# GaloisInc/pure-zlib

Hardware: AMD Instinct MI355X
Metric: decompressed GiB/s (whole node) on 64K level-6 zlib blobs; bit-exact vs ref (higher is better)
Workload: dtype u8

## Files before the change

pure_zlib_amd/csrc/inflate_core.h:

```cpp
#pragma once
#include <stddef.h>
#include <stdint.h>

#include "wave.h"

#if defined(PZG_PROFILE) && PZG_DEVICE_PASS && defined(PZG_PROFILE_HDR)
#define PZG_T0(var) const uint64_t var = __builtin_amdgcn_s_memtime()
#define PZG_ACC(slot, var) ((slot) >= 8 && (slot) <= 11 ? (void)var : (void)(prof[slot] += __builtin_amdgcn_s_memtime() - var))
#define PZG_ACCW(slot, var) ((void)var)
#define PZG_HACC(slot, var) prof[slot] += __builtin_amdgcn_s_memtime() - var
#elif defined(PZG_PROFILE) && PZG_DEVICE_PASS && defined(PZG_PROFILE_HOT)
#define PZG_T0(var) const uint64_t var = __builtin_amdgcn_s_memtime()
#define PZG_ACC(slot, var) ((slot) >= 8 && (slot) <= 11 ? (void)var : (void)(prof[slot] += __builtin_amdgcn_s_memtime() - var))
#define PZG_ACCW(slot, var) ((void)var)
#define PZG_HACC(slot, var)
#define PZG_HOT_ACC(slot, var) prof[slot] += __builtin_amdgcn_s_memtime() - var
#elif defined(PZG_PROFILE) && PZG_DEVICE_PASS
#define PZG_T0(var) const uint64_t var = __builtin_amdgcn_s_memtime()
#define PZG_ACC(slot, var) prof[slot] += __builtin_amdgcn_s_memtime() - var
#define PZG_ACCW(slot, var) (__builtin_amdgcn_s_waitcnt(0xc07f), prof[slot] += __builtin_amdgcn_s_memtime() - var)
#define PZG_HACC(slot, var)
#else
#define PZG_HACC(slot, var)
#define PZG_T0(var)
#define PZG_ACC(slot, var)
#define PZG_ACCW(slot, var)
#endif
#if defined(PZG_MARKS) && PZG_DEVICE_PASS
#define PZG_MARK(name) asm volatile("; ##MARK " name)
#else
#define PZG_MARK(name)
#endif
#ifndef PZG_HOT_ACC
#define PZG_HOT_ACC(slot, var)
#endif
#if defined(PZG_PROFILE) && PZG_DEVICE_PASS && defined(PZG_PROFILE_HOT)
#define PZG_SEQ_T0(var) uint64_t var = __builtin_amdgcn_s_memtime()
#define PZG_SEQ_ACC(slot, var) (__builtin_amdgcn_s_waitcnt(0x0070), prof[slot] += __builtin_amdgcn_s_memtime() - var, var = __builtin_amdgcn_s_memtime())
#else
#define PZG_SEQ_T0(var)
#define PZG_SEQ_ACC(slot, var)
#endif

#if defined(PZG_STATS) && !PZG_DEVICE_PASS
struct PzgStats { unsigned long long v[32]; };
extern PzgStats pzg_stats;
#define PZG_STAT(i, n) (pzg_stats.v[i] += (unsigned long long)(n))
#else
#define PZG_STAT(i, n) ((void)0)
#endif
#ifndef PZG_RES_HOT_LOOP
#define PZG_RES_HOT_LOOP 1
#endif
#ifndef PZG_WALK_UNROLL
#define PZG_WALK_UNROLL 8
#endif
#ifndef PZG_HOT_ALIGN
#define PZG_HOT_ALIGN 6
#endif
#ifndef PZG_WALK_EXIT_ALIGN
#define PZG_WALK_EXIT_ALIGN 2
#endif
#define PZG_STR2(x) #x
#define PZG_STR(x) PZG_STR2(x)

namespace pzg {

enum : int32_t {
    ST_OK = 0,
    ST_TRUNCATED = 1,
    ST_HDR_FCHECK = 2,
    ST_HDR_METHOD = 3,
    ST_HDR_WINDOW = 4,
    ST_FMT_LEN_NLEN = 5,
    ST_FMT_BTYPE = 6,
    ST_HUFF_BUILD = 7,
    ST_HUFF_EMPTY_TREE = 8,
    ST_HUFF_EMPTY_BRANCH = 9,
    ST_CHECKSUM = 10,
    ST_BAD_DISTANCE = 11,
    ST_BAD_LITLEN_SYMBOL = 12,
    ST_BAD_DIST_SYMBOL = 13,
    ST_OUT_TOO_SMALL = 14,
    ST_GZIP_HEADER = 18,
    ST_GZIP_ISIZE = 19,
    ST_DICT = 20,
    ST_SEGMENT = 21,
    ST_NEED_INPUT = 101,
    ST_OUT_FULL = 102,
    ST_RETRY_FULL_RING = 100,
    ST_BUNDLE_TODO = 103
};

enum { TREE_CODELEN = 0, TREE_LITLEN = 1, TREE_DIST = 2 };

#ifndef PZG_LIT_BITS
#define PZG_LIT_BITS 8
#endif
constexpr int LIT_BITS = PZG_LIT_BITS;
#ifndef PZG_SUB_ENTRIES
#define PZG_SUB_ENTRIES 252
#endif
constexpr uint32_t SUB_ENTRIES = PZG_SUB_ENTRIES;
static_assert(SUB_ENTRIES <= 256u, "K_SUB entries hold an 8-bit pool index");
#ifndef PZG_SUB_BITS_MAX
#define PZG_SUB_BITS_MAX 5
#endif
constexpr uint32_t SUB_BITS_MAX = PZG_SUB_BITS_MAX;
#ifndef PZG_SUB_MIN
#define PZG_SUB_MIN 3
#endif
constexpr uint32_t SUB_MIN_PREFIXES = PZG_SUB_MIN;
constexpr int DIST_BITS = 8;
constexpr int CL_BITS = 7;
constexpr uint32_t ADLER_MOD = 65521u;

constexpr int MAX_LIT_SYMS = 288;
constexpr int MAX_DIST_SYMS = 32 + 138;
constexpr int MAX_LENS = 288 + 32 + 138;

enum : uint32_t {
    K_LIT = 0,
    K_BASE = 1,
    K_EOB = 2,
    K_LONG = 3,
    K_EMPTY_BRANCH = 4,
    K_EMPTY_TREE = 5,
    K_BADSYM = 6,
// ... 1537 lines not shown
    template <bool FX>
    PZG_FN bool fill_queue()
    {
        while (__builtin_expect(br.window2_ok(), 1)) {
            if (__builtin_expect(window_append2<FX>(), 0)) return true;
            if (qn >= QHIGH) return false;
        }
        if (RES) {
            do {
                if (!br.window_ok() || window_append<FX>()) return true;
            } while (qn < QHIGH);
            return false;
        }
        do {
            if (window_append2<FX, true>()) return true;
        } while (qn < QHIGH);
        return false;
    }

    enum : uint32_t { HL_GENERAL = 1, HL_WINDOW = 2 };
    template <bool FX, int SUB>
    PZG_FN uint32_t hot_loop(LaneVec<uint32_t> &TK0, LaneVec<uint32_t> &TK1, uint64_t &S0, uint64_t &S1, uint32_t &k0, uint32_t &k1)
    {
        uint32_t why;
#if PZG_DEVICE_PASS && PZG_HOT_ALIGN
        asm volatile(".p2align " PZG_STR(PZG_HOT_ALIGN));
#endif
        for (;;) {
            if (qn < QHIGH) {
                if (__builtin_expect(!br.window2_ok(), 0)) {
                    why = HL_GENERAL;
                    break;
                }
                PZG_T0(thw);
                LaneVec<uint32_t> TB0, TB1;
                window2_decode<FX, false, SUB>(TB0, TK0, TB1, TK1);
                S0 = 0;
                S1 = 0;
                k1 = 0;
                PZG_STAT(0, 1);
                k0 = walk_half(TB0, 0u, S0);
                why = HL_WINDOW;
                if (__builtin_expect(k0 >= 64u, 0)) break;
                k1 = walk_half(TB1, k0, S1);
                if (__builtin_expect(k1 >= 64u, 0)) break;
                const uint32_t nt0 = popc64(S0), nt1 = popc64(S1);
                if (__builtin_expect((qn + nt0) + nt1 > QCAP, 0)) break;
                PZG_STAT(1, nt0 + nt1);
                queue_append(TK0, S0, nt0, TK1, S1, nt1);
                br.drop_short(k1 + 128u);
                PZG_HOT_ACC(8, thw);
                continue;
            }
            PZG_T0(the);
            if (emit_body<true>() != ST_OK) {
                why = HL_GENERAL;
                break;
            }
            PZG_HOT_ACC(9, the);
        }
#if PZG_DEVICE_PASS
        asm volatile("" : "+s"(why));
#endif
        return why;
    }


    static constexpr bool STRIPS = true;
#ifndef PZG_STRIP_TMAX
#define PZG_STRIP_TMAX 192
#endif
#ifndef PZG_STRIP_BACK
#define PZG_STRIP_BACK 1024
#endif
    static constexpr uint32_t STRIP_TMAX = PZG_STRIP_TMAX;
    static_assert(STRIP_TMAX % 16u == 0u && STRIP_TMAX <= 1008u, "region geometry");
    static constexpr bool SEQ_LROVF = STRIP_TMAX > 240u;
#ifndef PZG_SEQ_GROUP
#define PZG_SEQ_GROUP 8
#endif
#ifndef PZG_TOP_MOVES
#define PZG_TOP_MOVES 1
#endif
    static constexpr uint32_t SEQ_G = PZG_SEQ_GROUP;
    static constexpr uint32_t REG_LITA = 32u;
    static constexpr uint32_t REG_RECA = (REG_LITA + STRIP_TMAX + 4u * SEQ_G + 31u) & ~31u;
#ifndef PZG_REG_PAD
#define PZG_REG_PAD 0
#endif
    static constexpr uint32_t REG_BYTES = ((REG_RECA + 4u * STRIP_TMAX + 63u) & ~63u) + PZG_REG_PAD;
    static constexpr uint32_t PROF_OFF = 64u * (REG_BYTES / 4u) + 128u;
    static constexpr uint32_t STRIP_WORDS = PROF_OFF + 80u;
    static constexpr uint32_t PROF_MAGIC = 0x51DF0A7Eu;
#ifndef PZG_STRIP_PROFILE
#define PZG_STRIP_PROFILE 1
#endif
    static constexpr bool STRIP_PROFILE = PZG_STRIP_PROFILE != 0 && !RES;
#ifndef PZG_PROF_LIKELY
#define PZG_PROF_LIKELY(x) __builtin_expect(!!(x), 0)
#endif
    static constexpr uint32_t PROF_TGT = STRIP_TMAX * 3u / 4u;
#ifndef PZG_PROF_CMIN
#define PZG_PROF_CMIN 512
#endif
    static constexpr uint32_t PROF_CMIN = PZG_PROF_CMIN;
    static constexpr uint32_t PROF_HEAD = 2048u;
    static constexpr uint32_t STRIP_BACK = PZG_STRIP_BACK;
#ifndef PZG_STRIP_BACK_MIN
#define PZG_STRIP_BACK_MIN 256
#endif
    static constexpr uint32_t STRIP_BACK_MIN = PZG_STRIP_BACK_MIN < PZG_STRIP_BACK ? PZG_STRIP_BACK_MIN : PZG_STRIP_BACK;
    static constexpr uint32_t STRIP_BACK_DOWN = 32u, STRIP_BACK_UP = 256u;
#ifndef PZG_STRIP_CMIN
#define PZG_STRIP_CMIN 64
#endif
    static constexpr uint32_t STRIP_CMIN = PZG_STRIP_CMIN;
#ifndef PZG_STRIP_BACK_PER_C
#define PZG_STRIP_BACK_PER_C 2
#endif
    static constexpr uint32_t STRIP_BACK_PER_C = PZG_STRIP_BACK_PER_C;
#ifndef PZG_STRIP_ROUNDS
#define PZG_STRIP_ROUNDS 6
#endif
    static constexpr uint32_t STRIP_ROUNDS = PZG_STRIP_ROUNDS;
    static constexpr int STRIP_NA = -2;
    PZG_FN static constexpr uint32_t reg_rec(uint32_t k) { return k * (REG_BYTES / 4u) + REG_RECA / 4u; }
    PZG_FN static constexpr uint32_t reg_lit(uint32_t k) { return k * REG_BYTES + REG_LITA; }

    static constexpr uint32_t SEQ_NOMATCH = 0x80000000u;
    PZG_FN static uint32_t seq_nl(uint32_t rec) { return (rec >> 23) & 255u; }
    PZG_FN static uint32_t seq_len(uint32_t rec) { return (int32_t)rec < 0 ? 0u : ((rec >> 15) & 255u) + 3u; }
    PZG_FN static uint32_t seq_dist(uint32_t rec) { return (rec & 0x7fffu) + 1u; }

    PZG_FN uint32_t strip_load(uint32_t i) const
    {
#if PZG_DEVICE_PASS
        return __hip_atomic_load(strip + i, __ATOMIC_RELAXED, __HIP_MEMORY_SCOPE_AGENT);
#else
        return strip[i];
#endif
    }
    PZG_FN uint32_t lit_load32(uint32_t off) const
    {
        const uint8_t *p = reinterpret_cast<const uint8_t *>(strip) + off;
#if PZG_DEVICE_PASS
        return __hip_atomic_load(reinterpret_cast<const uint32_t *>(p), __ATOMIC_RELAXED, __HIP_MEMORY_SCOPE_AGENT);
#else
        uint32_t v;
        __builtin_memcpy(&v, p, 4);
        return v;
#endif
    }
    PZG_FN uint8_t lit_load8(uint32_t off) const
    {
        const uint8_t *p = reinterpret_cast<const uint8_t *>(strip) + off;
#if PZG_DEVICE_PASS
        return __hip_atomic_load(p, __ATOMIC_RELAXED, __HIP_MEMORY_SCOPE_AGENT);
#else
        return *p;
#endif
    }
    PZG_FN void strip_fence() const
    {
#if PZG_DEVICE_PASS
        asm volatile("s_waitcnt vmcnt(0)" ::: "memory");
#endif
// ... 756 lines not shown
        PZG_HOT_ACC(10, tsc);
        PZG_T0(tse);
        for (;;) {
            const uint32_t why = seq_hot();
            if (why == SQ_DONE) break;
            if (why == SQ_FLUSH) {
                flush_to(op & ~(uint64_t)15u);
                continue;
            }
            const int se = seq_solo();
            if (se) return se;
        }
        PZG_HOT_ACC(11, tse);
        strip_kill_window_state();
        return ST_OK;
    }
    PZG_FN void strip_kill_window_state()
    {
        PZG_LANES_BEGIN(j)
            PZG_LV(QT, j) = 0u;
            PZG_LV(pendF0, j) = 0;
            PZG_LV(pendF1, j) = 0;
        PZG_LANES_END
    }
#undef PZG_SR

#ifndef PZG_SEQ_GLIM
#define PZG_SEQ_GLIM 768
#endif
#ifndef PZG_SEQ_CAP
#define PZG_SEQ_CAP 32
#endif
    static constexpr uint32_t SEQ_GLIM = PZG_SEQ_GLIM;
    static constexpr uint32_t SEQ_CAP = PZG_SEQ_CAP;
    static_assert(SEQ_GLIM + SEQ_CAP + 3u + 128u <= 1024u && SEQ_GLIM >= 255u + SEQ_CAP, "far sources end a cache line or more below `flushed`; one sequence always fits");
    enum : uint32_t { SQ_OK = 0, SQ_DONE = 1, SQ_SOLO = 2, SQ_FLUSH = 3 };

    static constexpr uint32_t RING_OFF = (uint32_t)offsetof(WaveLds<RING_BITS>, ring);
    static constexpr uint32_t DUMP_REL = (uint32_t)(offsetof(WaveLds<RING_BITS>, dump) - offsetof(WaveLds<RING_BITS>, ring));
    struct Quad {
        uint8_t b[4];
    };
    template <uint32_t OFF>
    PZG_FN void lds_copy4x2(const LaneVec<uint32_t> &SM, const LaneVec<uint32_t> &DM, uint64_t m0, uint64_t m1)
    {
#if PZG_DEVICE_PASS
        static_assert(RING_OFF % 4u == 0u && OFF % 8u == 0u, "aligned dwords");
        uint32_t a, sh, d0, d1, d2, q0, q1, y0, y1;
        uint64_t sv;
        asm volatile("s_mov_b64 %9, exec\n\t"
                     "s_mov_b64 exec, %12\n\t"
                     "v_and_b32 %0, -4, %10\n\t"
                     "v_lshlrev_b32 %1, 3, %10\n\t"
                     "ds_read_b32 %2, %0 offset:%c14\n\tds_read_b32 %3, %0 offset:%c15\n\tds_read_b32 %4, %0 offset:%c16\n\t"
                     "s_waitcnt lgkmcnt(0)\n\t"
                     "v_alignbit_b32 %5, %3, %2, %1\n\t"
                     "v_alignbit_b32 %6, %4, %3, %1\n\t"
                     "v_lshrrev_b32 %7, 8, %5\n\t"
                     "v_lshrrev_b32 %8, 8, %6\n\t"
                     "s_mov_b64 exec, %13\n\t"
                     "ds_write_b8_d16_hi %11, %8 offset:%c24\n\tds_write_b8_d16_hi %11, %6 offset:%c23\n\tds_write_b8 %11, %8 offset:%c22\n\tds_write_b8 %11, %6 offset:%c21\n\t"
                     "s_mov_b64 exec, %12\n\t"
                     "ds_write_b8_d16_hi %11, %7 offset:%c20\n\tds_write_b8_d16_hi %11, %5 offset:%c19\n\tds_write_b8 %11, %7 offset:%c18\n\tds_write_b8 %11, %5 offset:%c17\n\t"
                     "s_mov_b64 exec, %9"
                     : "=&v"(a), "=&v"(sh), "=&v"(d0), "=&v"(d1), "=&v"(d2), "=&v"(q0), "=&v"(q1), "=&v"(y0), "=&v"(y1), "=&s"(sv)
                     : "v"(SM.v), "v"(DM.v), "s"(m0), "s"(m1), "n"(RING_OFF + OFF), "n"(RING_OFF + OFF + 4u), "n"(RING_OFF + OFF + 8u),
                       "n"(RING_OFF + OFF), "n"(RING_OFF + OFF + 1u), "n"(RING_OFF + OFF + 2u), "n"(RING_OFF + OFF + 3u), "n"(RING_OFF + OFF + 4u),
                       "n"(RING_OFF + OFF + 5u), "n"(RING_OFF + OFF + 6u), "n"(RING_OFF + OFF + 7u)
                     : "memory");
#else
        LaneVec<Quad> A, B;
        for (uint32_t j = 0; j < 64u; ++j)
            for (uint32_t t = 0; t < 4u; ++t) {
                if ((m0 >> j) & 1u) A.v[j].b[t] = L.ring[SM.v[j] + OFF + t];
                if ((m1 >> j) & 1u) B.v[j].b[t] = L.ring[SM.v[j] + OFF + 4u + t];
            }
        for (uint32_t j = 0; j < 64u; ++j)
            for (uint32_t t = 4u; t-- > 0u;) {
                if ((m1 >> j) & 1u) L.ring[DM.v[j] + OFF + 4u + t] = B.v[j].b[t];
                if ((m0 >> j) & 1u) L.ring[DM.v[j] + OFF + t] = A.v[j].b[t];
            }
#endif
    }
    PZG_FN void lds_copy_tail(const LaneVec<uint32_t> &ST, const LaneVec<uint32_t> &DT, uint64_t m4, const LaneVec<uint32_t> &S3,
                              const LaneVec<uint32_t> &D3, uint64_t m3)
    {
#if PZG_DEVICE_PASS
        uint32_t sa, da, a, sh, d0, d1, q, y;
        uint64_t sv;
        asm volatile("s_mov_b64 %8, exec\n\t"
                     "s_or_b64 exec, %13, %14\n\t"
                     "v_cndmask_b32_e64 %0, %11, %9, %13\n\t"
                     "v_cndmask_b32_e64 %1, %12, %10, %13\n\t"
                     "v_and_b32 %2, -4, %0\n\t"
                     "v_lshlrev_b32 %3, 3, %0\n\t"
                     "ds_read_b32 %4, %2 offset:%c15\n\tds_read_b32 %5, %2 offset:%c19\n\t"
                     "s_waitcnt lgkmcnt(0)\n\t"
                     "v_alignbit_b32 %6, %5, %4, %3\n\t"
                     "v_lshrrev_b32 %7, 8, %6\n\t"
                     "s_mov_b64 exec, %13\n\t"
                     "ds_write_b8_d16_hi %1, %7 offset:%c18\n\t"
                     "s_or_b64 exec, %13, %14\n\t"
                     "ds_write_b8_d16_hi %1, %6 offset:%c17\n\tds_write_b8 %1, %7 offset:%c16\n\tds_write_b8 %1, %6 offset:%c15\n\t"
                     "s_mov_b64 exec, %8"
                     : "=&v"(sa), "=&v"(da), "=&v"(a), "=&v"(sh), "=&v"(d0), "=&v"(d1), "=&v"(q), "=&v"(y), "=&s"(sv)
                     : "v"(ST.v), "v"(DT.v), "v"(S3.v), "v"(D3.v), "s"(m4), "s"(m3), "n"(RING_OFF), "n"(RING_OFF + 1u), "n"(RING_OFF + 2u), "n"(RING_OFF + 3u),
                       "n"(RING_OFF + 4u)
                     : "memory", "scc");
#else
        LaneVec<Quad> A, B;
        for (uint32_t j = 0; j < 64u; ++j)
            for (uint32_t t = 0; t < 4u; ++t) {
                if ((m4 >> j) & 1u) A.v[j].b[t] = L.ring[ST.v[j] + t];
                if (((m3 >> j) & 1u) && t < 3u) B.v[j].b[t] = L.ring[S3.v[j] + t];
            }
        for (uint32_t j = 0; j < 64u; ++j)
            for (uint32_t t = 4u; t-- > 0u;) {
                if (((m3 >> j) & 1u) && t < 3u) L.ring[D3.v[j] + t] = B.v[j].b[t];
                if ((m4 >> j) & 1u) L.ring[DT.v[j] + t] = A.v[j].b[t];
            }
#endif
    }
    PZG_FN void lds_put_bytes(const LaneVec<uint32_t> &A, const LaneVec<uint32_t> &X, uint64_t m0, uint64_t m1, uint64_t m2, uint64_t m3)
    {
#if PZG_DEVICE_PASS
        uint32_t y;
        uint64_t sv;
        asm volatile("s_mov_b64 %1, exec\n\t"
                     "s_mov_b64 exec, %7\n\t"
                     "v_lshrrev_b32 %0, 8, %3\n\t"
                     "ds_write_b8_d16_hi %2, %0 offset:%c11\n\t"
                     "s_mov_b64 exec, %6\n\t"
                     "ds_write_b8_d16_hi %2, %3 offset:%c10\n\t"
                     "s_mov_b64 exec, %5\n\t"
                     "v_lshrrev_b32 %0, 8, %3\n\t"
                     "ds_write_b8 %2, %0 offset:%c9\n\t"
                     "s_mov_b64 exec, %4\n\t"
                     "ds_write_b8 %2, %3 offset:%c8\n\t"
                     "s_mov_b64 exec, %1"
                     : "=&v"(y), "=&s"(sv)
                     : "v"(A.v), "v"(X.v), "s"(m0), "s"(m1), "s"(m2), "s"(m3), "n"(RING_OFF), "n"(RING_OFF + 1u), "n"(RING_OFF + 2u), "n"(RING_OFF + 3u)
                     : "memory");
#else
        for (uint32_t j = 0; j < 64u; ++j) {
            if ((m3 >> j) & 1u) L.ring[A.v[j] + 3u] = (uint8_t)(X.v[j] >> 24);
            if ((m2 >> j) & 1u) L.ring[A.v[j] + 2u] = (uint8_t)(X.v[j] >> 16);
            if ((m1 >> j) & 1u) L.ring[A.v[j] + 1u] = (uint8_t)(X.v[j] >> 8);
            if ((m0 >> j) & 1u) L.ring[A.v[j]] = (uint8_t)X.v[j];
        }
#endif
    }
    PZG_FN void lds_put_dword(const LaneVec<uint32_t> &A, const LaneVec<uint32_t> &X, uint64_t m)
    {
#if PZG_DEVICE_PASS
        uint32_t y;
        uint64_t sv;
        asm volatile("s_mov_b64 %1, exec\n\t"
                     "s_mov_b64 exec, %4\n\t"
                     "v_lshrrev_b32 %0, 8, %3\n\t"
                     "ds_write_b8_d16_hi %2, %0 offset:%c8\n\tds_write_b8_d16_hi %2, %3 offset:%c7\n\tds_write_b8 %2, %0 offset:%c6\n\tds_write_b8 %2, %3 offset:%c5\n\t"
                     "s_mov_b64 exec, %1"
                     : "=&v"(y), "=&s"(sv)
                     : "v"(A.v), "v"(X.v), "s"(m), "n"(RING_OFF), "n"(RING_OFF + 1u), "n"(RING_OFF + 2u), "n"(RING_OFF + 3u)
                     : "memory");
#else
        lds_put_bytes(A, X, m, m, m, m);
#endif
    }
    PZG_FN uint32_t far_off(uint32_t op32, uint32_t fdelta, uint32_t rel) const
    {
        return RES_HIST ? (op32 + rel) & HIST_MASK : 32768u + fdelta + rel;
    }
    PZG_FN uint32_t far_load32(uint32_t off) const
    {
#if PZG_DEVICE_PASS
        if (RES_HIST)
            return __hip_atomic_load(reinterpret_cast<const uint32_t *>(far_base + off), __ATOMIC_RELAXED, __HIP_MEMORY_SCOPE_AGENT);
#endif
        uint32_t v;
        __builtin_memcpy(&v, far_base + off, 4);
        return v;
    }
    PZG_FN uint8_t far_load8(uint32_t off) const
    {
#if PZG_DEVICE_PASS
        if (RES_HIST) return __hip_atomic_load(far_base + off, __ATOMIC_RELAXED, __HIP_MEMORY_SCOPE_AGENT);
#endif
        return far_base[off];
    }
    static constexpr uint32_t FAR_DUMMY = RES_HIST ? 0u : FAR_IDLE;
    struct SeqCopy {
        LaneVec<uint32_t> SM, DM, LEN, NB, ST, DT;
        uint64_t norm4, norm3, slow;
    };
    template <uint32_t T>
    PZG_FN void seq_copy_trips(const SeqCopy &c, uint64_t m4)
    {
        if constexpr (T < SEQ_CAP / 8u) {
            LaneVec<bool> A0, A1;
            PZG_LANES_BEGIN(j)
                PZG_LV(A0, j) = 2u * T < PZG_LV(c.NB, j);
                PZG_LV(A1, j) = 2u * T + 1u < PZG_LV(c.NB, j);
            PZG_LANES_END
            const uint64_t m0 = m4 & lanes_ballot(A0), m1 = m4 & lanes_ballot(A1);
            if (m0 == 0ull) return;
            lds_copy4x2<8u * T>(c.SM, c.DM, m0, m1);
            PZG_STAT(26, 1);
            seq_copy_trips<T + 1u>(c, m4);
        }
    }
    PZG_FN void seq_copy(const SeqCopy &c, uint64_t rdy)
    {
        const uint64_t m4 = rdy & c.norm4, m3 = rdy & c.norm3, sl = rdy & c.slow;
        if (m4 != 0ull) seq_copy_trips<0u>(c, m4);
        lds_copy_tail(c.ST, c.DT, m4, c.SM, c.DM, m3);
        if (__builtin_expect(sl != 0ull, 0)) {
            LaneVec<bool> ACT;
            LaneVec<uint32_t> X;
            for (uint32_t i = 0;; ++i) {
                PZG_LANES_BEGIN(j)
                    PZG_LV(ACT, j) = lane_bit(sl, j) & (i < PZG_LV(c.LEN, j));
                PZG_LANES_END
                if (lanes_ballot(ACT) == 0ull) break;
                PZG_LANES_BEGIN(j)
                    PZG_LV(X, j) = L.ring[(PZG_LV(c.SM, j) + i) & RMASK];
                PZG_LANES_END
                PZG_LANES_BEGIN(j)
                    ring_store(PZG_LV(ACT, j), (PZG_LV(c.DM, j) + i) & RMASK, (uint8_t)PZG_LV(X, j), j);
                PZG_LANES_END
                PZG_STAT(27, 1);
            }
        }
    }

    PZG_FN uint32_t seq_group()
    {
        const uint32_t n = s_qn;
        if (n == 0u) return SQ_DONE;
        if (__builtin_expect((uint32_t)(op - flushed) >= FLUSH_AT, 0)) {
            const uint64_t to = flushed + ((uint32_t)(op - flushed) & ~1023u);
            if (!out_aligned() || to > cap) return SQ_FLUSH;
            flush_span<true>(to);
        }
        PZG_SEQ_T0(tq);
        PZG_MARK("g.begin");
        const uint32_t op32 = (uint32_t)op;
        uint32_t op_hi = (uint32_t)(op >> 32);
#if PZG_DEVICE_PASS
        asm("" : "+s"(op_hi));
#endif
        const uint32_t hist = (op_hi | (op32 >> 20)) ? 0x100000u : op32 + (RING_BITS == 15 ? hist_extra : 0u);
        LaneVec<uint32_t> NL, LEN, DIST, ENDX, MO;
        PZG_LANES_BEGIN(j)
            const uint32_t rec = PZG_LV(QTN, j);
            const bool valid = j < n;
            const uint32_t nl = valid ? seq_nl(rec) : 0u, len = valid ? seq_len(rec) : 0u;
            PZG_LV(NL, j) = nl;
            PZG_LV(LEN, j) = len;
            PZG_LV(DIST, j) = seq_dist(rec);
            PZG_LV(ENDX, j) = (nl + len) | (nl << 16);
        PZG_LANES_END
        lanes_iscan_add(ENDX);
        LaneVec<bool> OVER, BAD, MIX, HASM;
        PZG_LANES_BEGIN(j)
            const uint32_t end = PZG_LV(ENDX, j) & 0xffffu, len = PZG_LV(LEN, j), m = end - len;
            PZG_LV(MO, j) = m;
            PZG_LV(OVER, j) = end > SEQ_GLIM;
            PZG_LV(HASM, j) = len != 0u;
            PZG_LV(BAD, j) = PZG_LV(DIST, j) > hist + m;
            PZG_LV(MIX, j) = (int32_t)(m - PZG_LV(DIST, j)) < (int32_t)(SEQ_GLIM - RING);
        PZG_LANES_END
        const uint64_t stopm = lanes_ballot(OVER) | (lanes_ballot(HASM) & (lanes_ballot(BAD) | (RING_BITS == 15 ? lanes_ballot(MIX) : 0ull)));
        const uint32_t v0 = stopm ? ctz64(stopm) : n;
        const uint32_t v = v0 < n ? v0 : n;
        if (__builtin_expect(v == 0u, 0)) return SQ_SOLO;
        const uint32_t endv = lane_get(ENDX, v - 1u), run = endv & 0xffffu, lend_v = endv >> 16;
        const uint64_t taken = v >= 64u ? ~0ull : bit_field_mask(v, 0u);
        PZG_STAT(20, 1);
        PZG_STAT(21, v);
        PZG_STAT(22, run);
        SeqCopy c;
        LaneVec<uint32_t> SEND;
        LaneVec<bool> B_LEN, B_NEAR, B_WD, B_WS, B_D16, B_OV, B_D4, B_BIG, B_L4, B_L3;
        PZG_LANES_BEGIN(j)
            const uint32_t len = PZG_LV(LEN, j), dist = PZG_LV(DIST, j), m = PZG_LV(MO, j);
            const int32_t srcr = (int32_t)(m - dist);
            const uint32_t dm = (op32 + m) & RMASK, sm = (dm - dist) & RMASK;
            PZG_LV(c.LEN, j) = len;
            PZG_LV(c.DM, j) = dm;
            PZG_LV(c.SM, j) = sm;
            PZG_LV(c.NB, j) = (len - 1u) >> 2;
            PZG_LV(c.ST, j) = sm + len - 4u;
            PZG_LV(c.DT, j) = dm + len - 4u;
            PZG_LV(B_LEN, j) = len != 0u;
            PZG_LV(B_NEAR, j) = srcr >= (int32_t)(run - RING);
            PZG_LV(B_WD, j) = dm + len > RING;
            PZG_LV(B_WS, j) = sm + len > RING;
            PZG_LV(B_D16, j) = dist < 16u;
            PZG_LV(B_OV, j) = len > dist;
            PZG_LV(B_D4, j) = dist < 4u;
            PZG_LV(B_BIG, j) = len > SEQ_CAP;
            PZG_LV(B_L4, j) = len >= 4u;
            PZG_LV(B_L3, j) = len == 3u;
            PZG_LV(SEND, j) = (uint32_t)srcr + (len < dist ? len : dist);
        PZG_LANES_END
        const uint64_t hasm = taken & lanes_ballot(B_LEN), coopm = hasm & lanes_ballot(B_BIG);
        const uint64_t nearx = HYBRID ? hasm & lanes_ballot(B_NEAR) & ~coopm : hasm & ~coopm;
        const uint64_t wrapd = lanes_ballot(B_WD);
        const uint64_t slowx = wrapd | lanes_ballot(B_WS) | (lanes_ballot(B_D16) & (lanes_ballot(B_OV) | lanes_ballot(B_D4)));
        c.slow = nearx & slowx;
        c.norm4 = nearx & ~slowx & lanes_ballot(B_L4);
        c.norm3 = nearx & ~slowx & lanes_ballot(B_L3);
        const uint64_t nearm = nearx | coopm;
#if defined(PZG_LAB) && defined(PZG_LAB_NOFAR)
        const uint64_t farm = 0ull;
#else
        const uint64_t farm = HYBRID ? hasm & ~nearx & ~coopm & far_okmask : 0ull;
#endif
        LaneVec<uint32_t> FO, FND, FX[4];
        uint64_t farn = farm & ~wrapd, fars = farm & wrapd;
        if (HYBRID && farm != 0ull) {
            PZG_STAT(25, 1);
            far_fence();
            const uint32_t fdelta = (uint32_t)(op - flushed);
            if (RES_HIST) {
                LaneVec<bool> HW;
                PZG_LANES_BEGIN(j)
                    PZG_LV(HW, j) = far_off(op32, fdelta, PZG_LV(MO, j) - PZG_LV(DIST, j)) + PZG_LV(c.LEN, j) + 3u > HIST_BYTES;
                PZG_LANES_END
                const uint64_t hw = lanes_ballot(HW);
                fars = farm & (wrapd | hw);
                farn = farm & ~(wrapd | hw);
            }
            PZG_LANES_BEGIN(j)
                const uint32_t len = PZG_LV(c.LEN, j), l4 = len >= 4u ? len - 4u : 0u;
                const uint32_t nd = mask_keep(farn, j, (len + 3u) >> 2), fo = far_off(op32, fdelta, PZG_LV(MO, j) - PZG_LV(DIST, j));
                PZG_LV(FND, j) = nd;
                PZG_LV(FO, j) = fo;
#pragma unroll
                for (uint32_t u = 0; u < 4u; ++u) {
                    const uint32_t off = 4u * u < l4 ? 4u * u : l4;
#if PZG_DEVICE_PASS
                    PZG_LV(FX[u], j) = far_load32(u < nd ? fo + off : FAR_DUMMY);
#else
                    PZG_LV(FX[u], j) = u < nd ? far_load32(fo + off) : 0u;
#endif
                }
            PZG_LANES_END
        }
        LaneVec<uint32_t> INFO, LOE, FLV, FLI, CL;
        PZG_LANES_BEGIN(j)
            PZG_LV(INFO, j) = PZG_LV(QINFO, j);
            PZG_LV(FLI, j) = (PZG_LV(QINFO, j) >> 8) & 63u;
            PZG_LV(LOE, j) = (PZG_LV(ENDX, j) >> 16) - PZG_LV(NL, j);
        PZG_LANES_END
        const uint32_t lc0 = s_lc, lit_a = reg_lit(lane_get(QINFO, 0u) & 255u);
        s_rd += v;
        const bool at_start = seq_refill();
        lanes_gather(FLV, LOE, FLI);
        PZG_LANES_BEGIN(j)
            PZG_LV(CL, j) = PZG_LV(LOE, j) + PZG_LV(NL, j) - PZG_LV(FLV, j) + (((PZG_LV(INFO, j) >> 16) & 1u) ? lc0 : 0u);
        PZG_LANES_END
        s_lc = at_start ? 0u : lane_get(CL, v - 1u);
        (void)lend_v;
        PZG_SEQ_ACC(12, tq);
        PZG_MARK("g.lits");
        LaneVec<uint32_t> LAD, DL, X0, X1;
        LaneVec<bool> B_NL, B_WL, B_N8, B_N5;
        PZG_LANES_BEGIN(j)
            const uint32_t nl = PZG_LV(NL, j);
            const uint32_t la = reg_lit(PZG_LV(INFO, j) & 255u) + PZG_LV(CL, j) - nl, dl = (op32 + PZG_LV(MO, j) - nl) & RMASK;
            PZG_LV(LAD, j) = la;
            PZG_LV(DL, j) = dl;
            PZG_LV(B_NL, j) = nl != 0u;
            PZG_LV(B_WL, j) = dl + nl > RING;
            PZG_LV(B_N8, j) = nl > 8u;
            PZG_LV(B_N5, j) = nl > 4u;
        PZG_LANES_END
        const uint64_t litm = taken & lanes_ballot(B_NL), wrapl = lanes_ballot(B_WL), fastl = litm & ~wrapl, slowl = litm & wrapl;
        const uint64_t morel = fastl & lanes_ballot(B_N8), fast5 = fastl & lanes_ballot(B_N5);
        PZG_LANES_BEGIN(j)
            const uint32_t nl = PZG_LV(NL, j), la = PZG_LV(LAD, j);
            const uint32_t off1 = nl - 4u < 4u ? nl - 4u : 4u;
            PZG_LV(X0, j) = lit_load32(mask_select(fastl, j, la, lit_a));
            PZG_LV(X1, j) = lit_load32(mask_select(fast5, j, la + off1, lit_a));
        PZG_LANES_END
        PZG_SEQ_ACC(13, tq);
        PZG_MARK("g.matches");
#if defined(PZG_STATS) && !PZG_DEVICE_PASS
        {
            uint32_t lvl[64], maxl = 0;
            for (uint32_t j = 0; j < 64u; ++j) {
                lvl[j] = 0;
                if (!((hasm >> j) & 1ull)) continue;
                const int32_t sj = (int32_t)(PZG_LV(MO, j) - PZG_LV(DIST, j)), ej = (int32_t)PZG_LV(SEND, j);
                uint32_t l = 1;
                for (uint32_t i = 0; i < j; ++i)
                    if (((hasm >> i) & 1ull) && (int32_t)PZG_LV(MO, i) < ej && (int32_t)(PZG_LV(MO, i) + PZG_LV(LEN, i)) > sj && lvl[i] + 1u > l) l = lvl[i] + 1u;
                lvl[j] = l;
                if (l > maxl) maxl = l;
            }
            PZG_STAT(28, maxl);
        }
#endif
        uint64_t pend = nearm;
        if (nearm != 0ull) {
            LaneVec<bool> RDY;
            PZG_LANES_BEGIN(j)
                PZG_LV(RDY, j) = (int32_t)PZG_LV(SEND, j) <= 0;
            PZG_LANES_END
            const uint64_t rdy = nearm & lanes_ballot(RDY) & ~coopm;
            seq_copy(c, rdy);
            pend &= ~rdy;
            PZG_STAT(23, 1);
        }
        PZG_SEQ_ACC(14, tq);
        {
            LaneVec<bool> G2, G3, G4;
            LaneVec<uint32_t> DL1;
            PZG_LANES_BEGIN(j)
                const uint32_t nl = PZG_LV(NL, j);
                PZG_LV(G2, j) = nl >= 2u;
                PZG_LV(G3, j) = nl >= 3u;
                PZG_LV(G4, j) = nl >= 4u;
                PZG_LV(DL1, j) = PZG_LV(DL, j) + (nl - 4u < 4u ? nl - 4u : 4u);
            PZG_LANES_END
            lds_put_bytes(DL, X0, fastl, fastl & lanes_ballot(G2), fastl & lanes_ballot(G3), fastl & lanes_ballot(G4));
            lds_put_dword(DL1, X1, fast5);
        }
        if (__builtin_expect(morel != 0ull, 0)) {
            LaneVec<bool> A0, A1;
            for (uint32_t i = 2u;; i += 2u) {
                PZG_LANES_BEGIN(j)
                    const uint32_t nd = (PZG_LV(NL, j) + 3u) >> 2;
                    PZG_LV(A0, j) = i < nd;
                    PZG_LV(A1, j) = i + 1u < nd;
                PZG_LANES_END
                const uint64_t a0 = morel & lanes_ballot(A0), a1 = morel & lanes_ballot(A1);
                if (a0 == 0ull) break;
                LaneVec<uint32_t> Y0, Y1, D0, D1;
                PZG_LANES_BEGIN(j)
                    const uint32_t l4 = PZG_LV(NL, j) - 4u, o0 = 4u * i < l4 ? 4u * i : l4, o1 = 4u * i + 4u < l4 ? 4u * i + 4u : l4;
                    PZG_LV(Y0, j) = lit_load32(mask_select(a0, j, PZG_LV(LAD, j) + o0, lit_a));
                    PZG_LV(Y1, j) = lit_load32(mask_select(a1, j, PZG_LV(LAD, j) + o1, lit_a));
                    PZG_LV(D0, j) = PZG_LV(DL, j) + o0;
                    PZG_LV(D1, j) = PZG_LV(DL, j) + o1;
                PZG_LANES_END
                lds_put_dword(D0, Y0, a0);
                lds_put_dword(D1, Y1, a1);
            }
        }
        if (__builtin_expect(slowl != 0ull, 0)) {
            LaneVec<bool> A0;
            for (uint32_t i = 0;; ++i) {
                PZG_LANES_BEGIN(j)
                    PZG_LV(A0, j) = i < PZG_LV(NL, j);
                PZG_LANES_END
                const uint64_t a0 = slowl & lanes_ballot(A0);
                if (a0 == 0ull) break;
                PZG_LANES_BEGIN(j)
                    const uint8_t b = lit_load8(mask_select(a0, j, PZG_LV(LAD, j) + i, lit_a));
                    ring_store(lane_bit(a0, j), (PZG_LV(DL, j) + i) & RMASK, b, j);
// ... 1140 lines not shown
```

Baseline: 336.5.

## Precompute copy source split and gate wrap/overlap classification on wave-uniform checks

Match copy setup now stores the source's aligned base and shift once, so the 4x2 LDS copy helper no longer recomputes alignment per trip. Length thresholds (>8, >12) are balloted up front, so the first copy trip and the tail (now merged for 4- and 3-byte tails) run without per-trip ballots. Wrap checks for destination and literals are skipped when a wave-uniform test shows the output run cannot cross the ring end. The overlap and short-distance checks are skipped when no lane has distance below 16. This trims VALU and ballot work in the sequence copy hot path, at the cost of more code paths and extra live registers.

```diff
diff --git a/pure_zlib_amd/csrc/inflate_core.h b/pure_zlib_amd/csrc/inflate_core.h
--- a/pure_zlib_amd/csrc/inflate_core.h
+++ b/pure_zlib_amd/csrc/inflate_core.h
@@ -43,7 +43,7 @@
 #endif
 
 #if defined(PZG_STATS) && !PZG_DEVICE_PASS
-struct PzgStats { unsigned long long v[32]; };
+struct PzgStats { unsigned long long v[40]; };
 extern PzgStats pzg_stats;
 #define PZG_STAT(i, n) (pzg_stats.v[i] += (unsigned long long)(n))
 #else
@@ -1747,6 +1747,15 @@
 #ifndef PZG_TOP_MOVES
 #define PZG_TOP_MOVES 1
 #endif
+#ifndef PZG_COPY_ONCE
+#define PZG_COPY_ONCE 1
+#endif
+#ifndef PZG_COPY_SPLIT
+#define PZG_COPY_SPLIT 1
+#endif
+#ifndef PZG_CLASS_GATES
+#define PZG_CLASS_GATES 1
+#endif
     static constexpr uint32_t SEQ_G = PZG_SEQ_GROUP;
     static constexpr uint32_t REG_LITA = 32u;
     static constexpr uint32_t REG_RECA = (REG_LITA + STRIP_TMAX + 4u * SEQ_G + 31u) & ~31u;
@@ -2669,6 +2678,37 @@
             }
 #endif
     }
+    template <uint32_t OFF>
+    PZG_FN void lds_copy4x2(const LaneVec<uint32_t> &SA, const LaneVec<uint32_t> &SH, const LaneVec<uint32_t> &DM, uint64_t m0, uint64_t m1)
+    {
+#if PZG_DEVICE_PASS
+        static_assert(RING_OFF % 4u == 0u && OFF % 8u == 0u, "aligned dwords");
+        uint32_t d0, d1, d2, q0, q1, y0, y1;
+        uint64_t sv;
+        asm volatile("s_mov_b64 %7, exec\n\t"
+                     "s_mov_b64 exec, %11\n\t"
+                     "ds_read_b32 %0, %8 offset:%c13\n\tds_read_b32 %1, %8 offset:%c14\n\tds_read_b32 %2, %8 offset:%c15\n\t"
+                     "s_waitcnt lgkmcnt(0)\n\t"
+                     "v_alignbit_b32 %3, %1, %0, %9\n\t"
+                     "v_alignbit_b32 %4, %2, %1, %9\n\t"
+                     "v_lshrrev_b32 %5, 8, %3\n\t"
+                     "v_lshrrev_b32 %6, 8, %4\n\t"
+                     "s_mov_b64 exec, %12\n\t"
+                     "ds_write_b8_d16_hi %10, %6 offset:%c23\n\tds_write_b8_d16_hi %10, %4 offset:%c22\n\tds_write_b8 %10, %6 offset:%c21\n\tds_write_b8 %10, %4 offset:%c20\n\t"
+                     "s_mov_b64 exec, %11\n\t"
+                     "ds_write_b8_d16_hi %10, %5 offset:%c19\n\tds_write_b8_d16_hi %10, %3 offset:%c18\n\tds_write_b8 %10, %5 offset:%c17\n\tds_write_b8 %10, %3 offset:%c16\n\t"
+                     "s_mov_b64 exec, %7"
+                     : "=&v"(d0), "=&v"(d1), "=&v"(d2), "=&v"(q0), "=&v"(q1), "=&v"(y0), "=&v"(y1), "=&s"(sv)
+                     : "v"(SA.v), "v"(SH.v), "v"(DM.v), "s"(m0), "s"(m1), "n"(RING_OFF + OFF), "n"(RING_OFF + OFF + 4u), "n"(RING_OFF + OFF + 8u),
+                       "n"(RING_OFF + OFF), "n"(RING_OFF + OFF + 1u), "n"(RING_OFF + OFF + 2u), "n"(RING_OFF + OFF + 3u), "n"(RING_OFF + OFF + 4u),
+                       "n"(RING_OFF + OFF + 5u), "n"(RING_OFF + OFF + 6u), "n"(RING_OFF + OFF + 7u)
+                     : "memory");
+#else
+        LaneVec<uint32_t> SM;
+        for (uint32_t j = 0; j < 64u; ++j) SM.v[j] = SA.v[j] + ((SH.v[j] >> 3) & 3u);
+        lds_copy4x2<OFF>(SM, DM, m0, m1);
+#endif
+    }
     PZG_FN void lds_copy_tail(const LaneVec<uint32_t> &ST, const LaneVec<uint32_t> &DT, uint64_t m4, const LaneVec<uint32_t> &S3,
                               const LaneVec<uint32_t> &D3, uint64_t m3)
     {
@@ -2708,6 +2748,37 @@
             }
 #endif
     }
+    PZG_FN void lds_copy_tail(const LaneVec<uint32_t> &ST, const LaneVec<uint32_t> &DT, uint64_t m4, uint64_t m43)
+    {
+#if PZG_DEVICE_PASS
+        uint32_t a, sh, d0, d1, q, y;
+        uint64_t sv;
+        asm volatile("s_mov_b64 %6, exec\n\t"
+                     "s_mov_b64 exec, %10\n\t"
+                     "v_and_b32 %0, -4, %7\n\t"
+                     "v_lshlrev_b32 %1, 3, %7\n\t"
+                     "ds_read_b32 %2, %0 offset:%c11\n\tds_read_b32 %3, %0 offset:%c15\n\t"
+                     "s_waitcnt lgkmcnt(0)\n\t"
+                     "v_alignbit_b32 %4, %3, %2, %1\n\t"
+                     "v_lshrrev_b32 %5, 8, %4\n\t"
+                     "s_mov_b64 exec, %9\n\t"
+                     "ds_write_b8_d16_hi %8, %5 offset:%c14\n\t"
+                     "s_mov_b64 exec, %10\n\t"
+                     "ds_write_b8_d16_hi %8, %4 offset:%c13\n\tds_write_b8 %8, %5 offset:%c12\n\tds_write_b8 %8, %4 offset:%c11\n\t"
+                     "s_mov_b64 exec, %6"
+                     : "=&v"(a), "=&v"(sh), "=&v"(d0), "=&v"(d1), "=&v"(q), "=&v"(y), "=&s"(sv)
+                     : "v"(ST.v), "v"(DT.v), "s"(m4), "s"(m43), "n"(RING_OFF), "n"(RING_OFF + 1u), "n"(RING_OFF + 2u), "n"(RING_OFF + 3u), "n"(RING_OFF + 4u)
+                     : "memory");
+#else
+        LaneVec<Quad> A;
+        for (uint32_t j = 0; j < 64u; ++j)
+            for (uint32_t t = 0; t < 4u; ++t)
+                if (((m43 >> j) & 1u) && (t < 3u || ((m4 >> j) & 1u))) A.v[j].b[t] = L.ring[ST.v[j] + t];
+        for (uint32_t j = 0; j < 64u; ++j)
+            for (uint32_t t = 4u; t-- > 0u;)
+                if (((m43 >> j) & 1u) && (t < 3u || ((m4 >> j) & 1u))) L.ring[DT.v[j] + t] = A.v[j].b[t];
+#endif
+    }
     PZG_FN void lds_put_bytes(const LaneVec<uint32_t> &A, const LaneVec<uint32_t> &X, uint64_t m0, uint64_t m1, uint64_t m2, uint64_t m3)
     {
 #if PZG_DEVICE_PASS
@@ -2777,8 +2848,19 @@
     }
     static constexpr uint32_t FAR_DUMMY = RES_HIST ? 0u : FAR_IDLE;
     struct SeqCopy {
+#if PZG_COPY_ONCE && PZG_COPY_SPLIT
+        LaneVec<uint32_t> SA, SH, DM, LEN, ST, DT;
+        uint64_t norm4, norm3, slow, q8, q12;
+        PZG_FN uint32_t sm(uint32_t j) const { return PZG_LV(SA, j) + ((PZG_LV(SH, j) >> 3) & 3u); }
+#elif PZG_COPY_ONCE
+        LaneVec<uint32_t> SM, DM, LEN, ST, DT;
+        uint64_t norm4, norm3, slow, q8, q12;
+        PZG_FN uint32_t sm(uint32_t j) const { return PZG_LV(SM, j); }
+#else
         LaneVec<uint32_t> SM, DM, LEN, NB, ST, DT;
         uint64_t norm4, norm3, slow;
+        PZG_FN uint32_t sm(uint32_t j) const { return PZG_LV(SM, j); }
+#endif
     };
     template <uint32_t T>
     PZG_FN void seq_copy_trips(const SeqCopy &c, uint64_t m4)
@@ -2786,12 +2868,21 @@
         if constexpr (T < SEQ_CAP / 8u) {
             LaneVec<bool> A0, A1;
             PZG_LANES_BEGIN(j)
+#if PZG_COPY_ONCE
+                PZG_LV(A0, j) = PZG_LV(c.LEN, j) > 8u * T + 4u;
+                PZG_LV(A1, j) = PZG_LV(c.LEN, j) > 8u * T + 8u;
+#else
                 PZG_LV(A0, j) = 2u * T < PZG_LV(c.NB, j);
                 PZG_LV(A1, j) = 2u * T + 1u < PZG_LV(c.NB, j);
+#endif
             PZG_LANES_END
             const uint64_t m0 = m4 & lanes_ballot(A0), m1 = m4 & lanes_ballot(A1);
             if (m0 == 0ull) return;
+#if PZG_COPY_ONCE && PZG_COPY_SPLIT
+            lds_copy4x2<8u * T>(c.SA, c.SH, c.DM, m0, m1);
+#else
             lds_copy4x2<8u * T>(c.SM, c.DM, m0, m1);
+#endif
             PZG_STAT(26, 1);
             seq_copy_trips<T + 1u>(c, m4);
         }
@@ -2799,8 +2890,21 @@
     PZG_FN void seq_copy(const SeqCopy &c, uint64_t rdy)
     {
         const uint64_t m4 = rdy & c.norm4, m3 = rdy & c.norm3, sl = rdy & c.slow;
+#if PZG_COPY_ONCE
+        if (m4 != 0ull) {
+#if PZG_COPY_SPLIT
+            lds_copy4x2<0u>(c.SA, c.SH, c.DM, m4, m4 & c.q8);
+#else
+            lds_copy4x2<0u>(c.SM, c.DM, m4, m4 & c.q8);
+#endif
+            PZG_STAT(26, 1);
+            if ((m4 & c.q12) != 0ull) seq_copy_trips<1u>(c, m4);
+        }
+        lds_copy_tail(c.ST, c.DT, m4, m4 | m3);
+#else
         if (m4 != 0ull) seq_copy_trips<0u>(c, m4);
         lds_copy_tail(c.ST, c.DT, m4, c.SM, c.DM, m3);
+#endif
         if (__builtin_expect(sl != 0ull, 0)) {
             LaneVec<bool> ACT;
             LaneVec<uint32_t> X;
@@ -2810,7 +2914,7 @@
                 PZG_LANES_END
                 if (lanes_ballot(ACT) == 0ull) break;
                 PZG_LANES_BEGIN(j)
-                    PZG_LV(X, j) = L.ring[(PZG_LV(c.SM, j) + i) & RMASK];
+                    PZG_LV(X, j) = L.ring[(c.sm(j) + i) & RMASK];
                 PZG_LANES_END
                 PZG_LANES_BEGIN(j)
                     ring_store(PZG_LV(ACT, j), (PZG_LV(c.DM, j) + i) & RMASK, (uint8_t)PZG_LV(X, j), j);
@@ -2869,23 +2973,36 @@
         SeqCopy c;
         LaneVec<uint32_t> SEND;
         LaneVec<bool> B_LEN, B_NEAR, B_WD, B_WS, B_D16, B_OV, B_D4, B_BIG, B_L4, B_L3;
+        const bool wrapg = !PZG_CLASS_GATES || (op32 & RMASK) + run > RING;
+        PZG_STAT(32, (op32 & RMASK) + run > RING ? 1 : 0);
+        PZG_STAT(33, (op32 & RMASK) + run == RING ? 1 : 0);
+        PZG_STAT(34, (op32 & RMASK) + run + 1u == RING ? 1 : 0);
+        PZG_STAT(35, (op32 & RMASK) + run == RING + 1u ? 1 : 0);
         PZG_LANES_BEGIN(j)
             const uint32_t len = PZG_LV(LEN, j), dist = PZG_LV(DIST, j), m = PZG_LV(MO, j);
             const int32_t srcr = (int32_t)(m - dist);
             const uint32_t dm = (op32 + m) & RMASK, sm = (dm - dist) & RMASK;
             PZG_LV(c.LEN, j) = len;
             PZG_LV(c.DM, j) = dm;
+#if PZG_COPY_ONCE && PZG_COPY_SPLIT
+            PZG_LV(c.SA, j) = sm & ~3u;
+            PZG_LV(c.SH, j) = sm << 3;
+#else
             PZG_LV(c.SM, j) = sm;
+#endif
+#if PZG_COPY_ONCE
+            const uint32_t l4 = (len > 4u ? len : 4u) - 4u;
+            PZG_LV(c.ST, j) = sm + l4;
+            PZG_LV(c.DT, j) = dm + l4;
+#else
             PZG_LV(c.NB, j) = (len - 1u) >> 2;
             PZG_LV(c.ST, j) = sm + len - 4u;
             PZG_LV(c.DT, j) = dm + len - 4u;
+#endif
             PZG_LV(B_LEN, j) = len != 0u;
             PZG_LV(B_NEAR, j) = srcr >= (int32_t)(run - RING);
-            PZG_LV(B_WD, j) = dm + len > RING;
             PZG_LV(B_WS, j) = sm + len > RING;
             PZG_LV(B_D16, j) = dist < 16u;
-            PZG_LV(B_OV, j) = len > dist;
-            PZG_LV(B_D4, j) = dist < 4u;
             PZG_LV(B_BIG, j) = len > SEQ_CAP;
             PZG_LV(B_L4, j) = len >= 4u;
             PZG_LV(B_L3, j) = len == 3u;
@@ -2893,8 +3010,34 @@
         PZG_LANES_END
         const uint64_t hasm = taken & lanes_ballot(B_LEN), coopm = hasm & lanes_ballot(B_BIG);
         const uint64_t nearx = HYBRID ? hasm & lanes_ballot(B_NEAR) & ~coopm : hasm & ~coopm;
-        const uint64_t wrapd = lanes_ballot(B_WD);
-        const uint64_t slowx = wrapd | lanes_ballot(B_WS) | (lanes_ballot(B_D16) & (lanes_ballot(B_OV) | lanes_ballot(B_D4)));
+        uint64_t wrapd = 0ull;
+        if (wrapg) {
+            PZG_LANES_BEGIN(j)
+                PZG_LV(B_WD, j) = PZG_LV(c.DM, j) + PZG_LV(c.LEN, j) > RING;
+            PZG_LANES_END
+            wrapd = lanes_ballot(B_WD);
+        }
+        const uint64_t d16 = lanes_ballot(B_D16);
+        uint64_t ovd4 = 0ull;
+        if (!PZG_CLASS_GATES || d16 != 0ull) {
+            PZG_LANES_BEGIN(j)
+                PZG_LV(B_OV, j) = PZG_LV(c.LEN, j) > PZG_LV(DIST, j);
+                PZG_LV(B_D4, j) = PZG_LV(DIST, j) < 4u;
+            PZG_LANES_END
+            ovd4 = lanes_ballot(B_OV) | lanes_ballot(B_D4);
+        }
+        const uint64_t slowx = wrapd | lanes_ballot(B_WS) | (d16 & ovd4);
+#if PZG_COPY_ONCE
+        {
+            LaneVec<bool> B_L8, B_L12;
+            PZG_LANES_BEGIN(j)
+                PZG_LV(B_L8, j) = PZG_LV(c.LEN, j) > 8u;
+                PZG_LV(B_L12, j) = PZG_LV(c.LEN, j) > 12u;
+            PZG_LANES_END
+            c.q8 = lanes_ballot(B_L8);
+            c.q12 = lanes_ballot(B_L12);
+        }
+#endif
         c.slow = nearx & slowx;
         c.norm4 = nearx & ~slowx & lanes_ballot(B_L4);
         c.norm3 = nearx & ~slowx & lanes_ballot(B_L3);
@@ -2960,11 +3103,17 @@
             PZG_LV(LAD, j) = la;
             PZG_LV(DL, j) = dl;
             PZG_LV(B_NL, j) = nl != 0u;
-            PZG_LV(B_WL, j) = dl + nl > RING;
             PZG_LV(B_N8, j) = nl > 8u;
             PZG_LV(B_N5, j) = nl > 4u;
         PZG_LANES_END
-        const uint64_t litm = taken & lanes_ballot(B_NL), wrapl = lanes_ballot(B_WL), fastl = litm & ~wrapl, slowl = litm & wrapl;
+        uint64_t wrapl = 0ull;
+        if (wrapg) {
+            PZG_LANES_BEGIN(j)
+                PZG_LV(B_WL, j) = PZG_LV(DL, j) + PZG_LV(NL, j) > RING;
+            PZG_LANES_END
+            wrapl = lanes_ballot(B_WL);
+        }
+        const uint64_t litm = taken & lanes_ballot(B_NL), fastl = litm & ~wrapl, slowl = litm & wrapl;
         const uint64_t morel = fastl & lanes_ballot(B_N8), fast5 = fastl & lanes_ballot(B_N5);
         PZG_LANES_BEGIN(j)
             const uint32_t nl = PZG_LV(NL, j), la = PZG_LV(LAD, j);
```

After: 339.3 (median of 6 runs). No clear change (+0.8%).
